# AILab-CVC/SEED-X

Hardware: AMD Instinct MI355X
Metric: end-to-end generations/sec (img-in -> txt + 1024px-img-out) (higher is better)
Workload: dtype fp16

## Files before the change

### seed-x_amd/csrc/gemm.hip

```cpp
#include "gemm_common.h"

namespace sxk_gemm {

template <typename TT, int BM, int BN, int WM, int WN, int NSTAGE, int AMODE>
__global__ __launch_bounds__(WM * WN * 64) void gemm_kernel(const GemmP p) {
#if defined(__HIP_DEVICE_COMPILE__)
  typedef typename TT::vec8 vec8;
  constexpr int NW = WM * WN;
  static_assert(NW == 4 || NW == 8, "4 or 8 waves per block");
  constexpr int TM = BM / WM, TN = BN / WN;
  constexpr int FM = TM / 16, FN = TN / 16;
  constexpr bool kGlu = (FN % 2 == 0);
  constexpr int BNP = (BN + 8 * NW - 1) / (8 * NW) * (8 * NW);
  constexpr int A_PER_WAVE = BM / (8 * NW);
  constexpr int B_PER_WAVE = BNP / (8 * NW);
  constexpr int LOADS = A_PER_WAVE + B_PER_WAVE;
  constexpr int A_BYTES = BM * 128, B_BYTES = BNP * 128, STAGE = A_BYTES + B_BYTES;
  static_assert(LOADS * (NSTAGE - 1) <= 63, "vmcnt range");
  extern __shared__ __attribute__((aligned(16))) unsigned char smem[];

  const int tid = threadIdx.x, lane = tid & 63;
  const int wave = __builtin_amdgcn_readfirstlane(tid >> 6);
  const int wm = wave / WN, wn = wave % WN;
  unsigned long long t_start = 0, t_first = 0, t_main = 0;
// ... 367 lines not shown
  SX_CHECK(a->M > 0 && a->N > 0 && a->K > 0, "sx_gemm: empty problem M=%d N=%d K=%d", a->M, a->N, a->K);
  SX_CHECK(a->K % 64 == 0, "sx_gemm: K=%d must be a multiple of 64 (pad the operand)", a->K);
  SX_CHECK(a->N % 16 == 0, "sx_gemm: N=%d must be a multiple of 16 (pad the weight)", a->N);
  SX_CHECK(!a->glu || a->N % 32 == 0, "sx_gemm: glu needs N %% 32 == 0");
  const int n_out = a->glu ? a->N / 2 : a->N;
  SX_CHECK(a->n_valid >= 0 && a->n_valid % 4 == 0 && a->n_valid <= n_out, "sx_gemm: n_valid=%d", a->n_valid);
  SX_CHECK(a->ldc >= (a->n_valid > 0 ? a->n_valid : n_out) && a->ldc % 4 == 0, "sx_gemm: ldc=%d invalid for n_out=%d",
           a->ldc, n_out);
  SX_CHECK(!a->residual || (a->ldr >= (a->n_valid > 0 ? a->n_valid : n_out) && a->ldr % 4 == 0), "sx_gemm: ldr=%d invalid", a->ldr);
  SX_CHECK(!a->bias2d || a->bias2d_rows > 0, "sx_gemm: bias2d_rows must be > 0");
  GemmP p;
  memset(&p, 0, sizeof(p));
  p.A = a->A; p.W = a->W; p.C = a->C; p.bias = a->bias; p.bias2d = a->bias2d; p.residual = a->residual;
  SX_CHECK(a->a_planes >= 0 && a->a_planes <= 2, "sx_gemm: a_planes=%d", a->a_planes);
  const int planes = a->a_planes == 2 ? 2 : 1;
  SX_CHECK(planes == 1 || (a->a_mode == SX_A_LINEAR && !ln), "sx_gemm: a_planes = 2 is for plain linear GEMMs");
  const int Kk = a->K * planes;
  p.M = a->M; p.N = a->N; p.K = Kk; p.Kw = a->K; p.ldc = a->ldc; p.ldr = a->ldr; p.res_mod = a->res_mod;
  p.n_valid = a->n_valid > 0 ? a->n_valid : n_out;
  p.bias2d_rows = a->bias2d_rows; p.out_dtype = a->out_dtype; p.act = a->act; p.glu = a->glu;
  p.ldb2 = a->ld_bias2d > 0 ? a->ld_bias2d : a->N;
  p.pad = 1;
  uint64_t a_bytes;
  if (a->a_mode == SX_A_CONV3X3) {
    SX_CHECK(a->Cin % 64 == 0 && a->K == 9 * a->Cin, "sx_gemm conv: Cin=%d K=%d", a->Cin, a->K);
    SX_CHECK(a->stride == 1 || a->stride == 2, "sx_gemm conv: stride");
    SX_CHECK(a->M == a->B * a->Hout * a->Wout, "sx_gemm conv: M != B*Hout*Wout");
    const int hv = a->upsample ? 2 * a->Hin : a->Hin, wv = a->upsample ? 2 * a->Win : a->Win;
    SX_CHECK(a->pad_mode == 0 || a->pad_mode == 1, "sx_gemm conv: pad_mode");
    const int padsum = a->pad_mode ? 1 : 2;
    SX_CHECK(a->Hout == (hv + padsum - 3) / a->stride + 1 && a->Wout == (wv + padsum - 3) / a->stride + 1,
             "sx_gemm conv: output geometry mismatch");
    p.pad = a->pad_mode ? 0 : 1;
    p.Hin = a->Hin; p.Win = a->Win; p.Cin = a->Cin; p.Hout = a->Hout; p.Wout = a->Wout;
    p.stride = a->stride; p.upsample = a->upsample;
    a_bytes = (uint64_t)a->B * a->Hin * a->Win * a->Cin * 2;
  } else {
    SX_CHECK(a->a_mode == SX_A_LINEAR, "sx_gemm: bad a_mode");
    a_bytes = (uint64_t)a->M * Kk * 2;
  }
  const uint64_t w_bytes = (uint64_t)a->N * a->K * 2;
  SX_CHECK(a_bytes < 0x7fffffffull && w_bytes < 0x7fffffffull, "sx_gemm: operand exceeds 2 GiB descriptor range");
  p.a_bytes = (unsigned)a_bytes;
  p.w_bytes = (unsigned)w_bytes;
  hipStream_t st = (hipStream_t)stream;
  p.res_init = (p.residual && p.act == SX_ACT_NONE && !p.glu) ? 1 : 0;
  if (ln) {
    SX_CHECK(a->a_mode == SX_A_LINEAR && !gn_stats, "sx_gemm_ln: linear GEMMs only");
    SX_CHECK(!(ln->row_stats_in && ln->row_stats_out), "sx_gemm_ln: a launch is a producer or a consumer, not both");
    if (ln->row_stats_out) {
      SX_CHECK(ln->x16_out && a->out_dtype == SX_F32 && !a->glu && a->act == SX_ACT_NONE && p.n_valid == a->N,
               "sx_gemm_ln producer: needs x16_out and a plain fp32 output of all N columns");
      SX_CHECK(ln->ld_x16 >= a->N && ln->ld_x16 % 4 == 0 && (((size_t)ln->x16_out) & 7) == 0, "sx_gemm_ln producer: ld_x16=%d", ln->ld_x16);
      p.ln_x16 = ln->x16_out; p.ln_ldx = ln->ld_x16; p.ln_out = ln->row_stats_out;
    } else {
      SX_CHECK(ln->colsum && ln->dim == a->K && ln->eps > 0.f, "sx_gemm_ln consumer: colsum / dim (= K) / eps");
      SX_CHECK(a->out_dtype == a->dtype && !a->residual && !a->bias2d, "sx_gemm_ln consumer: 16-bit output, no residual / bias2d");
      p.ln_in = ln->row_stats_in; p.ln_cs = ln->colsum; p.ln_eps = ln->eps; p.ln_inv_dim = 1.0f / (float)ln->dim;
    }
  }
  unsigned allow = 0x7f;
  if (ln) allow = 0;
  allow |= pp_supported(p, a->dtype, 256, a->a_mode) ? 0x80u : 0u;
  allow |= pp_supported(p, a->dtype, 320, a->a_mode) ? 0x100u : 0u;
  SX_CHECK(!(g_force_tile == 7 || g_force_tile == 8) || ((allow >> g_force_tile) & 1u),
           "sx_gemm: forced ping-pong tile has no kernel for this epilogue");
  if (ln) {
    const int plain = pick_tile(a->M, a->N, Kk, a->glu != 0, false, g_force_tile, 0x1ff);
    SX_CHECK((plain == 7 || plain == 8) && ((allow >> plain) & 1u),
             "sx_gemm_ln: M=%d N=%d K=%d does not run on a ping-pong tile with this epilogue (tile %d): keep sx_layernorm for it", a->M,
             a->N, a->K, plain);
    allow = 1u << plain;
  }
  const int cfg = pick_tile(a->M, a->N, Kk, a->glu != 0, a->a_mode == SX_A_CONV3X3, g_force_tile, allow);
  if (cfg == 7 || cfg == 8) {
    if (gn_stats && a->out_dtype == SX_F32 && !a->glu && a->act == SX_ACT_NONE && p.n_valid == a->N && a->N % gn_groups == 0 &&
        (a->N / gn_groups) % 2 == 0 && gn_rows % 256 == 0 && a->M % gn_rows == 0) {
      p.gn_stats = gn_stats; p.gn_groups = gn_groups; p.gn_cpg = a->N / gn_groups; p.gn_rows = gn_rows;
      *gn_fused = 1;
    }
    return launch_pp(p, a->dtype, cfg == 7 ? 256 : 320, a->a_mode, st);
  }
#define SX_GEMM_DISPATCH(TT)                                                  \
  switch (cfg) {                                                              \
    case 0: return launch_cfg<TT, 128, 128, 2, 2, 2>(p, a->a_mode, st);       \
    case 1: return launch_cfg<TT, 128, 80, 4, 1, 3>(p, a->a_mode, st);        \
    case 2: return launch_cfg<TT, 64, 128, 2, 2, 3>(p, a->a_mode, st);        \
    case 3: return launch_cfg<TT, 64, 64, 2, 2, 3>(p, a->a_mode, st);         \
    case 4: return launch_cfg<TT, 256, 256, 2, 4, 2>(p, a->a_mode, st);       \
    case 5: return launch_cfg<TT, 256, 320, 2, 4, 2>(p, a->a_mode, st);       \
    default: return launch_cfg<TT, 256, 160, 4, 2, 2>(p, a->a_mode, st);      \
  }
  if (a->dtype == SX_BF16) { SX_GEMM_DISPATCH(BF16) } else { SX_GEMM_DISPATCH(F16) }
#undef SX_GEMM_DISPATCH
}
```

### seed-x_amd/csrc/gemm_pp.hip

```cpp
#include "gemm_common.h"
#include <type_traits>

namespace sxk_gemm {

#define SX_A_CONV3X3_UP 2

#define PP_SYNC()                            \
  do {                                       \
    __builtin_amdgcn_sched_barrier(0);       \
    __builtin_amdgcn_s_barrier();            \
    __builtin_amdgcn_sched_barrier(0);       \
  } while (0)

template <typename TT, int BN, int AMODE, bool OUT32, int ACT, bool GLU, int LN = 0>
__global__ __launch_bounds__(512) void gemm_pp_kernel(const GemmP p) {
#if defined(__HIP_DEVICE_COMPILE__)
  typedef typename TT::vec8 vec8;
  static_assert(LN != 2 || (OUT32 && !GLU && ACT == SX_ACT_NONE), "the LayerNorm producer is the plain fp32-output epilogue");
  constexpr int BM = 256, TN = BN / 4, FN = TN / 16, FM = 8, FH = 4;
  constexpr int NB = BN / 64;
  constexpr int C1 = NB - 3, C2 = 3;
  constexpr int WAITN = 4 + NB;
  constexpr int A_BYTES = BM * 128, STAGE = A_BYTES + BN * 128;
  static_assert(!GLU || FN % 2 == 0, "GLU pairs n-fragments");
  static_assert(BN == 256 || BN == 320, "ping-pong tiles are 256x256 and 256x320");
  extern __shared__ __attribute__((aligned(16))) unsigned char smem[];

  const int tid = threadIdx.x, lane = tid & 63;
  const int wave = __builtin_amdgcn_readfirstlane(tid >> 6);
  const int g = wave >> 2, wc = wave & 3;
  unsigned long long t_start = 0, t_first = 0, t_main = 0;
  if (p.dbg) t_start = __builtin_amdgcn_s_memtime();

  int tile_m, tile_n;
  if (!tile_coords(p, blockIdx.x, gridDim.x, tile_m, tile_n)) return;
  const int m0 = tile_m * BM, n0 = tile_n * BN;

  double ln_s1 = 0.0, ln_s2 = 0.0;
  if constexpr (LN == 1) {
    if (tid < BM) {
      const int m = m0 + tid < p.M ? m0 + tid : p.M - 1;
      ln_s1 = p.ln_in[2 * (size_t)m];
      ln_s2 = p.ln_in[2 * (size_t)m + 1];
    }
  }
  __amdgpu_buffer_rsrc_t rA = __builtin_amdgcn_make_buffer_rsrc((void*)p.A, 0, (int)p.a_bytes, 0x00020000);
  __amdgpu_buffer_rsrc_t rW = __builtin_amdgcn_make_buffer_rsrc((void*)p.W, 0, (int)p.w_bytes, 0x00020000);

  const int rl = lane >> 3;
  const unsigned gchunk = ((lane & 7) ^ rl) << 4;
  unsigned a_off[4], a_msk[4];
  int a_lrow[4];
#pragma unroll
  for (int s = 0; s < 4; ++s) {
    a_lrow[s] = g * 128 + (s >> 1) * 64 + ((2 * wave + (s & 1)) & 7) * 8;
    const int row = m0 + a_lrow[s] + rl;
    if (AMODE == SX_A_LINEAR) {
      a_off[s] = (row < p.M) ? (unsigned)row * (unsigned)p.K * 2u + gchunk : 0xC0000000u;
      a_msk[s] = 0;
    } else {
      const int hw = p.Hout * p.Wout;
      const int b = row / hw, rem = row - b * hw;
      const int oy = rem / p.Wout, ox = rem - oy * p.Wout;
      const int Hv = p.upsample ? 2 * p.Hin : p.Hin, Wv = p.upsample ? 2 * p.Win : p.Win;
      const int vy = oy * p.stride - p.pad, vx = ox * p.stride - p.pad;
      unsigned msk = 0;
#pragma unroll
      for (int t = 0; t < 9; ++t) {
        const int iy = vy + t / 3, ix = vx + t % 3;
        if (row < p.M && iy >= 0 && iy < Hv && ix >= 0 && ix < Wv) msk |= 1u << t;
      }
      int sy = vy, sx = vx;
      if (AMODE == SX_A_CONV3X3_UP) {
        sy = oy >> 1; sx = ox >> 1;
        msk |= (unsigned)(oy & 1) << 9 | (unsigned)(ox & 1) << 10;
      }
      a_off[s] = (unsigned)(((b * p.Hin + sy) * p.Win + sx) * p.Cin) * 2u + gchunk;
      a_msk[s] = msk;
    }
  }
  unsigned w_off[NB];
#pragma unroll
  for (int i = 0; i < NB; ++i) {
    const int row = n0 + (wave * NB + i) * 8 + rl;
    w_off[i] = (row < p.N) ? (unsigned)row * (unsigned)p.Kw * 2u + gchunk : 0xC0000000u;
  }
  const int cpt = (AMODE != SX_A_LINEAR) ? p.Cin / 64 : 1;
  const int nkt = p.K / 64;
  const int nkw = p.Kw / 64;

  struct Tap { int cc, dy, dx; };
  auto tap_next = [&](Tap& t) {
    if (++t.cc == cpt) { t.cc = 0; if (++t.dx == 3) { t.dx = 0; ++t.dy; } }
  };

  auto koff_of = [&](int kt) -> unsigned { return (kt < nkt) ? (unsigned)kt * 128u : 0x80000000u; };
  auto koff_w = [&](int kt) -> unsigned { return (kt < nkt) ? (unsigned)(kt >= nkw ? kt - nkw : kt) * 128u : 0x80000000u; };
  auto dma_a = [&](int s, int buf, int kt, const Tap& t) {
    unsigned voff;
    if (AMODE == SX_A_LINEAR) {
      voff = a_off[s] + koff_of(kt);
    } else {
      const int tap = t.dy * 3 + t.dx;
      const bool ok = ((a_msk[s] >> tap) & 1u) != 0 && kt < nkt;
      unsigned o;
      if (AMODE == SX_A_CONV3X3_UP) {
        const int ry = ((int)((a_msk[s] >> 9) & 1u) + t.dy - 1) >> 1, rx = ((int)((a_msk[s] >> 10) & 1u) + t.dx - 1) >> 1;
        o = a_off[s] + (unsigned)((ry * p.Win + rx) * p.Cin) * 2u + (unsigned)t.cc * 128u;
      } else {
        o = a_off[s] + (unsigned)(((t.dy * p.Win + t.dx) * p.Cin + t.cc * 64) * 2);
      }
      voff = ok ? o : 0x80000000u;
    }
    __builtin_amdgcn_raw_ptr_buffer_load_lds(rA, SX_LDS_PTR(smem + buf * STAGE + a_lrow[s] * 128), 16, voff, 0, 0, 0);
  };
  auto dma_w = [&](int i, int buf, int kt) {
    __builtin_amdgcn_raw_ptr_buffer_load_lds(rW, SX_LDS_PTR(smem + buf * STAGE + A_BYTES + (wave * NB + i) * 1024), 16,
                                             w_off[i] + koff_w(kt), 0, 0, 0);
  };
  auto issue_x = [&](int buf, int kt, const Tap& t) {
    dma_a(0, buf, kt, t);
    dma_a(1, buf, kt, t);
#pragma unroll
    for (int i = 0; i < C1; ++i) dma_w(i, buf, kt);
  };
  auto issue_y = [&](int buf, int kt) {
// ... 112 lines not shown
    if (kt + 1 < nkt) ktile(std::integral_constant<int, 1>{}, kt + 1);
  }
  if (g == 0) PP_SYNC();
  wait_vmcnt<0>();

  if (p.dbg) t_main = __builtin_amdgcn_s_memtime();
  int ncol[FN], nout[FN];
  bool nok[FN];
  f32x4_t bv[FN];
#pragma unroll
  for (int i = 0; i < FN; ++i) {
    const int nb = n0 + wc * TN + i * 16;
    ncol[i] = nb + lq;
    nout[i] = GLU ? (nb >> 1) + lq : ncol[i];
    nok[i] = ncol[i] < p.N && nout[i] < p.n_valid && !(GLU && (i & 1));
    if (ncol[i] >= p.N) ncol[i] = p.N - 4;
    if (nout[i] + 4 > p.ldc) nout[i] = 0;
    bv[i] = (f32x4_t){0.f, 0.f, 0.f, 0.f};
  }
  if (p.bias) {
#pragma unroll
    for (int i = 0; i < FN; ++i) bv[i] = *(const f32x4_t*)(p.bias + ncol[i]);
  }
  const bool b2_uniform = p.bias2d && (m0 / p.bias2d_rows) == ((m0 + BM - 1 < p.M ? m0 + BM - 1 : p.M - 1) / p.bias2d_rows);
  if (b2_uniform) {
    const float* b2 = p.bias2d + (size_t)(m0 / p.bias2d_rows) * p.ldb2;
#pragma unroll
    for (int i = 0; i < FN; ++i) bv[i] += *(const f32x4_t*)(b2 + ncol[i]);
  }
  const bool b2_rows = p.bias2d && !b2_uniform;
  const bool res_late = p.residual && !p.res_init;
  const bool wide = !OUT32 && !GLU && (p.ldc & 7) == 0 && (((size_t)p.C) & 15) == 0;
  bool pair_ok[(FN + 1) / 2];
#pragma unroll
  for (int i = 0; i < (FN + 1) / 2; ++i) {
    const int lim = p.n_valid < p.N ? p.n_valid : p.N;
    pair_ok[i] = (2 * i + 1 < FN) && (n0 + wc * TN + i * 32 + 32 <= lim);
  }
  const bool glu_wide = GLU && !OUT32 && (p.ldc & 7) == 0 && (((size_t)p.C) & 15) == 0 &&
                        ((n0 + wc * TN) >> 1) + 32 <= (p.n_valid < (p.N >> 1) ? p.n_valid : (p.N >> 1));
  auto act1 = [&](f32x4_t x) -> f32x4_t {
    if (ACT == SX_ACT_GELU) {
      const f32x2_t g0 = gelu_erf2((f32x2_t){x[0], x[1]}), g1 = gelu_erf2((f32x2_t){x[2], x[3]});
      return (f32x4_t){g0[0], g0[1], g1[0], g1[1]};
    } else if (ACT == SX_ACT_SILU) {
      return (f32x4_t){silu_f(x[0]), silu_f(x[1]), silu_f(x[2]), silu_f(x[3])};
    }
    return x;
  };
  auto pack4 = [&](f32x4_t x) -> u32x2_t {
    u32x2_t o;
    o[0] = pack2<TT>(x[0], x[1]);
    o[1] = pack2<TT>(x[2], x[3]);
    return o;
  };
  f32x4_t lcs[LN == 1 ? FN : 1];
  if constexpr (LN == 1) {
#pragma unroll
    for (int i = 0; i < FN; ++i) lcs[i] = *(const f32x4_t*)(p.ln_cs + ncol[i]);
  }
  float lsum[LN == 2 ? FM : 1], lsq[LN == 2 ? FM : 1];
  const bool gn = OUT32 && p.gn_stats != nullptr;
  float gsl[FN], gql[FN], gsh[FN], gqh[FN];
#pragma unroll
  for (int i = 0; i < FN; ++i) gsl[i] = gql[i] = gsh[i] = gqh[i] = 0.f;
#pragma unroll
  for (int j = 0; j < FM; ++j) {
    const int m = m0 + g * 128 + j * 16 + (lane & 15);
    const bool mok = m < p.M;
    const int mc = mok ? m : p.M - 1;
    f32x4_t v[FN];
    if constexpr (LN == 1) {
      const f32x2_t ab = *(const f32x2_t*)(ln_lds + 2 * (g * 128 + j * 16 + (lane & 15)));
#pragma unroll
      for (int i = 0; i < FN; ++i) v[i] = acc[i][j] * ab[0] + (lcs[i] * ab[1] + bv[i]);
    } else {
#pragma unroll
      for (int i = 0; i < FN; ++i) v[i] = acc[i][j] + bv[i];
    }
    if (b2_rows) {
      const float* b2 = p.bias2d + (size_t)(mc / p.bias2d_rows) * p.ldb2;
#pragma unroll
      for (int i = 0; i < FN; ++i) v[i] += *(const f32x4_t*)(b2 + ncol[i]);
    }
    if (GLU) {
#pragma unroll
      for (int i = 0; i + 1 < FN; i += 2) {
        const f32x4_t gt = act1(v[i + 1]);
        v[i] = v[i] * gt;
      }
    } else if (ACT != SX_ACT_NONE) {
#pragma unroll
      for (int i = 0; i < FN; ++i) v[i] = act1(v[i]);
    }
    if (res_late) {
      const float* rr = p.residual + (size_t)(p.res_mod ? (mc % p.res_mod) : mc) * p.ldr;
#pragma unroll
      for (int i = 0; i < FN; ++i) {
        if (GLU && (i & 1)) continue;
        const int c = (nout[i] + 4 <= p.ldr) ? nout[i] : 0;
        v[i] += *(const f32x4_t*)(rr + c);
      }
    }
    if (OUT32) {
#pragma unroll
      for (int i = 0; i < FN; ++i)
        if (mok && nok[i]) *(f32x4_t*)((float*)p.C + (size_t)m * p.ldc + nout[i]) = v[i];
      if constexpr (LN == 2) {
        float s1 = 0.f, s2 = 0.f;
#pragma unroll
        for (int i = 0; i < FN; ++i) {
          if (mok && nok[i]) {
            s1 += (v[i][0] + v[i][1]) + (v[i][2] + v[i][3]);
            s2 += (v[i][0] * v[i][0] + v[i][1] * v[i][1]) + (v[i][2] * v[i][2] + v[i][3] * v[i][3]);
          }
        }
        lsum[j] = s1;
        lsq[j] = s2;
        const bool xwide = (p.ln_ldx & 7) == 0 && (((size_t)p.ln_x16) & 15) == 0;
#pragma unroll
        for (int i = 0; i < FN; ++i) {
          if ((i & 1) == 0 && i + 1 < FN && xwide && pair_ok[i >> 1]) {
            const u32x2_t o0 = pack4(v[i]), o1 = pack4(v[i + 1]);
            const auto w0 = __builtin_amdgcn_permlane16_swap(o0[0], o1[0], false, false);
            const auto w1 = __builtin_amdgcn_permlane16_swap(o0[1], o1[1], false, false);
            if (mok) {
              const u32x4_t w4 = {w0[0], w1[0], w0[1], w1[1]};
              const int q = lane >> 4;
              const int col = n0 + wc * TN + i * 16 + (q & 1) * 16 + (q >> 1) * 8;
              *(u32x4_t*)((unsigned short*)p.ln_x16 + (size_t)m * p.ln_ldx + col) = w4;
// ... 19 lines not shown
          const u32x2_t o0 = pack4(v[0]), o1 = pack4(v[2]);
          const auto s0 = __builtin_amdgcn_permlane16_swap(o0[0], o1[0], false, false);
          const auto s1 = __builtin_amdgcn_permlane16_swap(o0[1], o1[1], false, false);
          if (mok) {
            const u32x4_t w4 = {s0[0], s1[0], s0[1], s1[1]};
            const int q = lane >> 4;
            const int col = ((n0 + wc * TN) >> 1) + (q & 1) * 16 + (q >> 1) * 8;
            *(u32x4_t*)((unsigned short*)p.C + (size_t)m * p.ldc + col) = w4;
          }
          continue;
        }
      }
#pragma unroll
      for (int i = 0; i < FN; ++i) {
        if (GLU && (i & 1)) continue;
        if (!GLU && wide && (i & 1) == 0 && i + 1 < FN && pair_ok[i >> 1]) {
          const u32x2_t o0 = pack4(v[i]), o1 = pack4(v[i + 1]);
          const auto s0 = __builtin_amdgcn_permlane16_swap(o0[0], o1[0], false, false);
          const auto s1 = __builtin_amdgcn_permlane16_swap(o0[1], o1[1], false, false);
          if (mok) {
            const u32x4_t w4 = {s0[0], s1[0], s0[1], s1[1]};
            const int q = lane >> 4;
            const int col = n0 + wc * TN + i * 16 + (q & 1) * 16 + (q >> 1) * 8;
            *(u32x4_t*)((unsigned short*)p.C + (size_t)m * p.ldc + col) = w4;
          }
          continue;
        }
        if (!GLU && wide && (i & 1) && pair_ok[i >> 1]) continue;
        if (mok && nok[i]) *(u32x2_t*)((unsigned short*)p.C + (size_t)m * p.ldc + nout[i]) = pack4(v[i]);
      }
    }
  }
  if constexpr (LN == 2) {
    float* racc = (float*)smem;
    __syncthreads();
#pragma unroll
    for (int j = 0; j < FM; ++j) {
      float s1 = lsum[j], s2 = lsq[j];
      s1 += __shfl_xor(s1, 16, 64); s2 += __shfl_xor(s2, 16, 64);
      s1 += __shfl_xor(s1, 32, 64); s2 += __shfl_xor(s2, 32, 64);
      if (lane < 16) *(f32x2_t*)(racc + ((size_t)(wc * BM + g * 128 + j * 16 + lane)) * 2) = (f32x2_t){s1, s2};
    }
    __syncthreads();
    if (tid < BM && m0 + tid < p.M) {
      float s1 = 0.f, s2 = 0.f;
#pragma unroll
      for (int w = 0; w < 4; ++w) { s1 += racc[(w * BM + tid) * 2]; s2 += racc[(w * BM + tid) * 2 + 1]; }
      atomicAdd(&p.ln_out[2 * (size_t)(m0 + tid)], (double)s1);
      atomicAdd(&p.ln_out[2 * (size_t)(m0 + tid) + 1], (double)s2);
    }
  }
  if (OUT32 && gn) {
// ... 77 lines not shown
  if (p.glu) {
    if (out32) return -1;
    if (p.act == SX_ACT_GELU) return 2;
    if (p.act == SX_ACT_SILU) return 3;
    return -1;
  }
  if (p.act == SX_ACT_NONE) return out32 ? 4 : 0;
  if (p.act == SX_ACT_GELU && !out32) return 1;
  return -1;
}

bool pp_supported(const GemmP& p, int dtype, int bn, int a_mode) {
  const int e = epi_code(p, dtype);
  if (e < 0) return false;
  if (p.ln_in && !(a_mode == SX_A_LINEAR && (e == 0 || e == 2) && !p.ln_out)) return false;
  if (p.ln_out && !(a_mode == SX_A_LINEAR && e == 4 && !p.gn_stats)) return false;
  if (bn == 320 && (e == 2 || e == 3)) return false;
  if (a_mode == SX_A_CONV3X3 && !(e == 0 || e == 4)) return false;
  if (a_mode == SX_A_CONV3X3 && p.upsample && !(p.stride == 1 && p.pad == 1)) return false;
  return bn == 256 || bn == 320;
}

template <typename TT>
static int launch_t(const GemmP& p, int dtype, int bn, int a_mode, hipStream_t st) {
  const int e = epi_code(p, dtype);
#define PP_CASE(BNV, AM, O32, ACTV, GLUV) return launch_one<TT, BNV, AM, O32, ACTV, GLUV>(p, st)
  if (p.ln_in) {
    if (e == 2) return launch_one<TT, 256, SX_A_LINEAR, false, SX_ACT_GELU, true, 1>(p, st);
    if (bn == 256) return launch_one<TT, 256, SX_A_LINEAR, false, SX_ACT_NONE, false, 1>(p, st);
    return launch_one<TT, 320, SX_A_LINEAR, false, SX_ACT_NONE, false, 1>(p, st);
  }
  if (p.ln_out) {
    if (bn == 256) return launch_one<TT, 256, SX_A_LINEAR, true, SX_ACT_NONE, false, 2>(p, st);
    return launch_one<TT, 320, SX_A_LINEAR, true, SX_ACT_NONE, false, 2>(p, st);
  }
  if (a_mode == SX_A_LINEAR) {
    if (bn == 256) {
      switch (e) {
        case 0: PP_CASE(256, SX_A_LINEAR, false, SX_ACT_NONE, false);
        case 1: PP_CASE(256, SX_A_LINEAR, false, SX_ACT_GELU, false);
        case 2: PP_CASE(256, SX_A_LINEAR, false, SX_ACT_GELU, true);
        case 3: PP_CASE(256, SX_A_LINEAR, false, SX_ACT_SILU, true);
        case 4: PP_CASE(256, SX_A_LINEAR, true, SX_ACT_NONE, false);
      }
    } else {
      switch (e) {
        case 0: PP_CASE(320, SX_A_LINEAR, false, SX_ACT_NONE, false);
        case 1: PP_CASE(320, SX_A_LINEAR, false, SX_ACT_GELU, false);
// ... 39 lines not shown
```

### seed-x_amd/ops.py

```python
import contextlib
import ctypes as C
import gc
import math

import os

import torch

from . import _lib
from ._lib import (SX_A_CONV3X3, SX_A_LINEAR, SX_ACT_GELU, SX_ACT_NONE, SX_ACT_SILU, SX_BF16, SX_F16, SX_F32,
                   AttnArgs, AttnSmallArgs, GemmArgs, GemvArgs, check)

_DT = {torch.float16: SX_F16, torch.bfloat16: SX_BF16, torch.float32: SX_F32}
_TD = {v: k for k, v in _DT.items()}
ACT = {None: SX_ACT_NONE, "none": SX_ACT_NONE, "gelu": SX_ACT_GELU, "silu": SX_ACT_SILU}


def dt_code(dtype):
    return _DT[dtype]


def _stream():
    return C.c_void_p(torch.cuda.current_stream().cuda_stream)

# ... 111 lines not shown
    args.bias2d_rows = bias2d_rows
    args.dtype = _DT[a.dtype]
    args.out_dtype = _DT[out_dtype]
    args.act = ACT[act]
    args.glu = 1 if glu else 0
    args.a_mode = SX_A_LINEAR
    args.a_planes = a_planes
    if ln_emit is not None or ln_apply is not None:
        assert gn is None and not (ln_emit is not None and ln_apply is not None)
        la = _lib.GemmLnArgs()
        if ln_emit is not None:
            assert ln_emit.x16.shape == (M, N) and ln_emit.x16.dtype == a.dtype and ln_emit.stats.shape[0] == M
            la.x16_out, la.ld_x16, la.row_stats_out = ln_emit.x16.data_ptr(), ln_emit.x16.stride(0), ln_emit.stats.data_ptr()
        else:
            rows, colsum, eps = ln_apply
            assert rows.stats.shape[0] == M and colsum.dtype == torch.float32 and colsum.numel() == N and colsum.is_contiguous()
            la.row_stats_in, la.colsum, la.dim, la.eps = rows.stats.data_ptr(), colsum.data_ptr(), K, float(eps)
        check(lib.sx_gemm_ln(C.byref(args), C.byref(la), _stream()), "sx_gemm_ln")
        return out
    _launch_gemm(lib, args, gn, "sx_gemm")
    return out


def conv3x3(x, w, bias=None, bias2d=None, residual=None, stride=1, upsample=False, out_dtype=None, act=None,
            n_valid=0, pad_mode=0, gn=None):
    lib = _lib.load()
    assert x.dim() == 4 and x.is_contiguous() and w.is_contiguous()
    B, H, W, Cin = x.shape
    Cout, K = w.shape
    assert K == 9 * Cin
    hv, wv = (2 * H, 2 * W) if upsample else (H, W)
    padsum = 1 if pad_mode else 2
    Hout, Wout = (hv + padsum - 3) // stride + 1, (wv + padsum - 3) // stride + 1
    M = B * Hout * Wout
    out_dtype = out_dtype or x.dtype
    n_store = n_valid if n_valid else Cout
    out = torch.empty((M, n_store), dtype=out_dtype, device=x.device)
    args = GemmArgs()
    args.A, args.W, args.C = x.data_ptr(), w.data_ptr(), out.data_ptr()
    args.bias = _f32c(bias).data_ptr() if bias is not None else None
    args.n_valid = n_valid
    if bias2d is not None:
        assert bias2d.dtype == torch.float32 and bias2d.stride(-1) == 1 and bias2d.shape == (B, Cout)
        args.bias2d = bias2d.data_ptr()
        args.bias2d_rows = Hout * Wout
        args.ld_bias2d = bias2d.stride(0)
    if residual is not None:
        assert residual.dtype == torch.float32 and residual.stride(-1) == 1
        args.residual = residual.data_ptr()
        args.ldr = residual.stride(0)
    args.M, args.N, args.K = M, Cout, K
    args.ldc = n_store
    args.dtype = _DT[x.dtype]
    args.out_dtype = _DT[out_dtype]
    args.act = ACT[act]
    args.a_mode = SX_A_CONV3X3
    args.B, args.Hin, args.Win, args.Cin, args.Hout, args.Wout = B, H, W, Cin, Hout, Wout
    args.stride = stride
    args.upsample = 1 if upsample else 0
    args.pad_mode = pad_mode
    _launch_gemm(lib, args, gn, "sx_gemm(conv3x3)")
    return out.view(B, Hout * Wout, n_store)


def pack_decode_tiles(w):
    N, K = w.shape
    assert N % 16 == 0 and K % 32 == 0
    return w.view(N // 16, 16, K // 32, 32).permute(0, 2, 1, 3).contiguous().view(N, K)


def pack_decode_tiles20(w):
    N, K = w.shape
    assert N % 20 == 0 and K % 32 == 0
    return w.view(N // 20, 20, K // 32, 32).permute(0, 2, 1, 3).contiguous().view(N, K)


def _fp8_row_order(codes):
    K = codes.shape[-1]
    return codes.reshape(*codes.shape[:-1], K // 64, 2, 4, 8).transpose(-3, -2).reshape(*codes.shape[:-1], K // 64, 64)


def pack_decode_tiles_fp8(codes):
# ... 928 lines not shown
```

### seed-x_amd/unet.py

```python
import math
import os
import types

import torch

from . import ops
from .llama import glu_pack_rows

LN_FOLD = os.environ.get("SX_LN_FOLD", "1") != "0"

SDXL_BASE_CONFIG = dict(in_channels=4, out_channels=4, block_out_channels=(320, 640, 1280), layers_per_block=2,
                        down_attn=(False, True, True), up_attn=(True, True, False), transformer_layers=(1, 2, 10),
                        heads=(5, 10, 20), cross_attention_dim=2048, addition_time_embed_dim=256, pooled_dim=1280,
                        norm_groups=32, sample_size=128)


class UNetOutput:
    def __init__(self, sample):
        self.sample = sample


class UNet2DConditionModel:
    def __init__(self, comm=None, **cfg):
        from .parallel import Comm
# ... 165 lines not shown
        for i, co in enumerate(boc):
            blk = dict(res=[], attn=[], down=None)
            for j in range(c["layers_per_block"]):
                blk["res"].append(resnet(f"down_blocks.{i}.resnets.{j}"))
                if c["down_attn"][i]:
                    blk["attn"].append(transformer(f"down_blocks.{i}.attentions.{j}", c["transformer_layers"][i], c["heads"][i]))
            if i != len(boc) - 1:
                n = f"down_blocks.{i}.downsamplers.0.conv"
                blk["down"] = (conv16(n + ".weight"), f32(n + ".bias"))
            P["down"].append(blk)
        P["mid"] = dict(res=[resnet("mid_block.resnets.0")], attn=[transformer("mid_block.attentions.0", c["transformer_layers"][-1], c["heads"][-1])])
        P["mid"]["res"].append(resnet("mid_block.resnets.1"))
        P["up"] = []
        rh, rl = list(reversed(c["heads"])), list(reversed(c["transformer_layers"]))
        for i in range(len(boc)):
            blk = dict(res=[], attn=[], up=None)
            for j in range(c["layers_per_block"] + 1):
                blk["res"].append(resnet(f"up_blocks.{i}.resnets.{j}"))
                if c["up_attn"][i]:
                    blk["attn"].append(transformer(f"up_blocks.{i}.attentions.{j}", rl[i], rh[i]))
            if i != len(boc) - 1:
                n = f"up_blocks.{i}.upsamplers.0.conv"
                blk["up"] = (conv16(n + ".weight"), f32(n + ".bias"))
            P["up"].append(blk)
        P["norm_out"] = (f32("conv_norm_out.weight"), f32("conv_norm_out.bias"))
        wo = conv16("conv_out.weight")
        wop = torch.zeros(16, wo.shape[1], dtype=dt, device=dev)
        wop[:wo.shape[0]] = wo
        bo = torch.zeros(16, dtype=torch.float32, device=dev)
        bo[:wo.shape[0]] = f32("conv_out.bias")
        P["conv_out_w"], P["conv_out_b"] = wop, bo
        ws = [sd[n + ".time_emb_proj.weight"].detach().to(dev, dt) for n in self._temb_names]
        bs = [sd[n + ".time_emb_proj.bias"].detach().to(dev, torch.float32) for n in self._temb_names]
        P["temb_w"], P["temb_b"] = torch.cat(ws, 0).contiguous(), torch.cat(bs, 0).contiguous()
        off, P["temb_off"] = 0, {}
        for n, w_ in zip(self._temb_names, ws):
            P["temb_off"][n] = (off, w_.shape[0])
            off += w_.shape[0]
        self._P = P
        self._sd = None
        return P

    def _gn(self, x, gb, eps, silu, Hc, Wc, want_raw=False, x2=None, stats=None):
        G, dt = self.cfg["norm_groups"], self.dtype
        return ops.groupnorm(x, gb[0], gb[1], G, eps, silu, dt, want_raw=want_raw, x2=x2, comm=self.comm, hw_total=Hc * Wc,
                             stats=stats)

    def _gn_slot(self, B, HW):
        if self._gn_arena is None:
            return None
        i = self._gn_next
        self._gn_next += 1
        if i >= self._gn_arena.shape[0]:
            return None
        return ops.GnStats(self._gn_arena[i], self.cfg["norm_groups"], HW)

    def _conv(self, h16, B, Hc, Wc, w, bias=None, bias2d=None, residual=None, stride=1, upsample=False, n_valid=0, gn=None):
        tp = self.comm.world
        Cin = h16.shape[-1]
        if tp == 1:
            return ops.conv3x3(h16.view(B, Hc, Wc, Cin), w, bias=bias, bias2d=bias2d, residual=residual, stride=stride,
                               upsample=upsample, out_dtype=torch.float32, n_valid=n_valid, gn=gn)
        from . import seqpar
        Hl = Hc // tp
        Co = n_valid or w.shape[0]
        if stride == 2:
            xin = seqpar.with_halo(h16, self.comm, Hl, Wc, left_col=True, bottom=False)
            out = ops.conv3x3(xin, w, bias=bias, bias2d=bias2d, stride=2, pad_mode=1, out_dtype=torch.float32)
            assert residual is None
            return out.view(B, (Hl // 2) * (Wc // 2), Co)
        xin = seqpar.with_halo(h16, self.comm, Hl, Wc)
        out = ops.conv3x3(xin, w, bias=bias, bias2d=bias2d, upsample=upsample, out_dtype=torch.float32, n_valid=n_valid)
        f = 2 if upsample else 1
        out = out.view(B, f * (Hl + 2), f * Wc, Co)[:, f:f * (Hl + 1)].reshape(B, f * Hl * f * Wc, Co).contiguous()
        if residual is not None:
            out = ops.add(out, residual.reshape(out.shape).contiguous())
        return out

    def _resnet(self, r, x, B, Hc, Wc, temb_all, skip=None, st_in=None):
        Ci = x.shape[-1] + (skip.shape[-1] if skip is not None else 0)
        if "ws" in r:
            h, raw = self._gn(x, r["n1"], 1e-5, True, Hc, Wc, want_raw=True, x2=skip)
        else:
            assert skip is None
            h = self._gn(x, r["n1"], 1e-5, True, Hc, Wc, stats=st_in)
# ... 150 lines not shown
            for j, r in enumerate(blk["res"]):
                x, st = self._resnet(r, x, B, Hc, Wc, temb_all, st_in=st)
                if blk["attn"]:
                    x, st = self._transformer(blk["attn"][j], x, B, ctx[ti], Hc, Wc, st_in=st)
                    ti += 1
                skips.append((x, Hc, Wc))
            if blk["down"] is not None:
                st = self._gn_slot(B, (Hc // 2) * (Wc // 2))
                x = self._conv(ops.cast(x, dt), B, Hc, Wc, blk["down"][0], bias=blk["down"][1], stride=2, gn=st)
                Hc, Wc = Hc // 2, Wc // 2
                skips.append((x, Hc, Wc))
        x, st = self._resnet(P["mid"]["res"][0], x, B, Hc, Wc, temb_all, st_in=st)
        x, st = self._transformer(P["mid"]["attn"][0], x, B, ctx[ti], Hc, Wc, st_in=st)
        ti += 1
        x, st = self._resnet(P["mid"]["res"][1], x, B, Hc, Wc, temb_all, st_in=st)
        for blk in P["up"]:
            for j, r in enumerate(blk["res"]):
                s, _, _ = skips.pop()
                x, st = self._resnet(r, x.contiguous(), B, Hc, Wc, temb_all, skip=s)
                if blk["attn"]:
                    x, st = self._transformer(blk["attn"][j], x, B, ctx[ti], Hc, Wc, st_in=st)
                    ti += 1
            if blk["up"] is not None:
                x = self._conv(ops.cast(x, dt), B, Hc, Wc, blk["up"][0], bias=blk["up"][1], upsample=True)
                Hc, Wc = Hc * 2, Wc * 2
                st = None
        h = self._gn(x, P["norm_out"], 1e-5, True, Hc, Wc, stats=st)
        self._gn_arena = None
        self._on_mark = None
        nv = 4 if c["out_channels"] == 4 else 0
        out = self._conv(h, B, Hc, Wc, P["conv_out_w"], bias=P["conv_out_b"], n_valid=nv)
        out = out.view(B, -1, out.shape[-1])
        if tp > 1:
            out = seqpar.gather_rows(out, self.comm)
            if not torch.cuda.is_current_stream_capturing():
                self.comm.check()
        return out

    def forward(self, sample, timestep, encoder_hidden_states, added_cond_kwargs=None, cross_attention_kwargs=None,
                return_dict=True, **_):
        self._pack()
        assert added_cond_kwargs is not None and "text_embeds" in added_cond_kwargs and "time_ids" in added_cond_kwargs
        B, Cin, H, W = sample.shape
        assert Cin == self.cfg["in_channels"]
        dev = self.device
        t = torch.as_tensor(timestep, dtype=torch.float32, device=dev).reshape(-1)
        t = t.expand(B).contiguous() if t.numel() == 1 else t
# ... 11 lines not shown
```

### seed-x_amd/vae.py

```python
import json
import math
import os
from types import SimpleNamespace

import torch

from . import ops

EPS = 1e-6


def pack_planes(w32, taps=1, role="w"):
    w3 = w32.reshape(w32.shape[0], taps, -1)
    hi = w3.to(torch.bfloat16)
    lo = (w3 - hi.float()).to(torch.bfloat16)
    planes = [hi, lo, hi] if role == "w" else [hi, hi, lo]
    return torch.cat(planes, dim=2).reshape(w32.shape[0], -1).contiguous()


class DecoderOutput:
    def __init__(self, sample):
        self.sample = sample


# ... 208 lines not shown

        lc, boc = c.latent_channels, c.block_out_channels
        assert lc == 4, "post_quant_conv / conv_in packing assumes 4 latent channels"
        top = boc[-1]
        P = {}
        bpq = torch.zeros(16, dtype=torch.float32, device=dev)
        bpq[:lc] = f32("post_quant_conv.bias")
        P["pq"] = (padded(f32("post_quant_conv.weight").reshape(lc, lc), 16, 64), bpq)
        self.cin_kpad = (9 * lc + 63) // 64 * 64
        P["conv_in"] = (padded(conv32("decoder.conv_in.weight"), top, self.cin_kpad), f32("decoder.conv_in.bias"))
        a = "decoder.mid_block.attentions.0."
        P["mid"] = dict(r0=resnet("decoder.mid_block.resnets.0"), r1=resnet("decoder.mid_block.resnets.1"),
                        gn=(f32(a + "group_norm.weight"), f32(a + "group_norm.bias")),
                        wq=lin16(a + "to_q.weight"), bq=f32(a + "to_q.bias"),
                        wk=lin16(a + "to_k.weight"), bk=f32(a + "to_k.bias"),
                        wv=lin16(a + "to_v.weight", role="a"), bv=f32(a + "to_v.bias"),
                        wo=lin16(a + "to_out.0.weight"), bo=f32(a + "to_out.0.bias"))
        P["up"] = []
        for i in range(len(boc)):
            blk = dict(res=[resnet(f"decoder.up_blocks.{i}.resnets.{j}") for j in range(c.layers_per_block + 1)], up=None)
            if i != len(boc) - 1:
                n = f"decoder.up_blocks.{i}.upsamplers.0.conv"
                blk["up"] = (conv16(n + ".weight"), f32(n + ".bias"))
            P["up"].append(blk)
        P["norm_out"] = (f32("decoder.conv_norm_out.weight"), f32("decoder.conv_norm_out.bias"))
        wo = conv32("decoder.conv_out.weight")
        bo = torch.zeros(16, dtype=torch.float32, device=dev)
        bo[:wo.shape[0]] = f32("decoder.conv_out.bias")
        if two:
            w16 = torch.zeros(16, 9, wo.shape[1] // 9, dtype=torch.float16, device=dev)
            w16[:wo.shape[0]] = wo.reshape(wo.shape[0], 9, -1).to(torch.float16)
            P["conv_out"] = (torch.cat([w16, w16], dim=2).reshape(16, -1).contiguous(), bo)
        else:
            P["conv_out"] = (padded(wo, 16, wo.shape[1], taps=9), bo)
        P["p_out"] = (2 if two else 3) if split else 1
        P["two"] = two
        if self.has_encoder:
            E = {}
            ci = c.in_channels
            self.enc_kpad = (9 * ci + 63) // 64 * 64
            E["conv_in"] = (padded(conv32("encoder.conv_in.weight"), boc[0], self.enc_kpad), f32("encoder.conv_in.bias"))
            E["down"] = []
            for i in range(len(boc)):
                blk = dict(res=[resnet(f"encoder.down_blocks.{i}.resnets.{j}") for j in range(c.layers_per_block)], down=None)
                if i != len(boc) - 1:
                    n = f"encoder.down_blocks.{i}.downsamplers.0.conv"
# ... 80 lines not shown
    def _im2col(self, x, kpad):
        if not self.split:
            return ops.im2col3x3_small(x, kpad, self.operand_dtype)
        pl = ops.split_bf16(x.view(-1, 4))
        hi, lo = (ops.im2col3x3_small(ops.cast(pl[:, a:a + 4].contiguous(), torch.float32).view(x.shape), kpad,
                                      torch.bfloat16) for a in (0, 8))
        return torch.cat([hi, hi, lo], dim=1)

    def _decode_one(self, z_nchw):
        P, c, f32 = self._P, self.config, torch.float32
        _, lc, h, w = z_nchw.shape
        zp = ops.nchw_to_nhwc(z_nchw, ld=64)
        x = ops.gemm(self._A(zp.view(-1, 64)), P["pq"][0], bias=P["pq"][1], out_dtype=f32, n_valid=4)
        col = self._im2col(x.view(1, h, w, lc), self.cin_kpad)
        x = ops.gemm(col, P["conv_in"][0], bias=P["conv_in"][1], out_dtype=f32).view(1, h * w, -1)
        x = self._resnet(P["mid"]["r0"], x, h, w)
        x = self._mid_attention(P["mid"], x)
        x = self._resnet(P["mid"]["r1"], x, h, w)
        H, W = h, w
        for blk in P["up"]:
            for r in blk["res"]:
                x = self._resnet(r, x, H, W)
            if blk["up"] is not None:
                x = ops.conv3x3(self._A(x).view(1, H, W, -1), blk["up"][0], bias=blk["up"][1], upsample=True, out_dtype=f32)
                H, W = 2 * H, 2 * W
        hN = self._gn(x, P["norm_out"], True, planes=P["p_out"])
        y = self._conv(P["p_out"], hN.view(1, H, W, -1), P["conv_out"][0], bias=P["conv_out"][1], out_dtype=f32,
                       n_valid=4)
        return ops.nhwc_to_nchw(y, c.out_channels, H, W)

    @torch.no_grad()
    def decode(self, z, return_dict=True, generator=None):
        self._pack()
        z = z.to(device=self.device, dtype=torch.float32)
        ops.OPERAND_PLANES = 3 if self.split else 1
        try:
            out = torch.cat([self._decode_one(z[b:b + 1].contiguous()) for b in range(z.shape[0])], dim=0)
        finally:
            ops.OPERAND_PLANES = 1
        return DecoderOutput(out) if return_dict else (out,)

    def _encode_one(self, img_nchw):
        P, c, f32 = self._P, self.config, torch.float32
        E = P["enc"]
        _, ci, H, W = img_nchw.shape
        nb = len(c.block_out_channels)
        assert H % (1 << (nb - 1)) == 0 and W % (1 << (nb - 1)) == 0
# ... 37 lines not shown
```

Baseline: 1.330.

## Decompose upsample+3x3 conv into four 2x2 sub-pixel phase convolutions

Nearest-neighbour 2x upsample followed by a 3x3 conv is rewritten as four phase-specific 2x2 convolutions over the low-resolution input. The kernel gains a new A-mode that gathers 4 taps instead of 9 and selects a per-phase weight slice. Output rows are scattered to their interleaved positions. This cuts the reduction length and the A-gather work for the upsampler convs in the UNet and VAE decoder. In exchange it adds pre-summed weights, which change rounding, plus extra weight memory and a constraint that the tile not straddle phases.

After: 1.352 (median of 6 runs). 1.7% higher.

```diff
diff --git a/seed-x_amd/csrc/gemm.hip b/seed-x_amd/csrc/gemm.hip
--- a/seed-x_amd/csrc/gemm.hip
+++ b/seed-x_amd/csrc/gemm.hip
@@ -413,9 +413,18 @@
   p.ldb2 = a->ld_bias2d > 0 ? a->ld_bias2d : a->N;
   p.pad = 1;
   uint64_t a_bytes;
+  const bool phases = a->a_mode == SX_A_CONV3X3 && a->upsample == 2;
   if (a->a_mode == SX_A_CONV3X3) {
-    SX_CHECK(a->Cin % 64 == 0 && a->K == 9 * a->Cin, "sx_gemm conv: Cin=%d K=%d", a->Cin, a->K);
+    SX_CHECK(a->upsample >= 0 && a->upsample <= 2, "sx_gemm conv: upsample=%d", a->upsample);
+    SX_CHECK(a->Cin % 64 == 0 && a->K == (phases ? 4 : 9) * a->Cin, "sx_gemm conv: Cin=%d K=%d", a->Cin, a->K);
     SX_CHECK(a->stride == 1 || a->stride == 2, "sx_gemm conv: stride");
+    if (phases) {
+      SX_CHECK(a->stride == 1 && a->pad_mode == 0, "sx_gemm conv: upsample = 2 is stride 1, pad 1");
+      SX_CHECK((int64_t)a->B * a->Hin * a->Win % 256 == 0,
+               "sx_gemm conv: upsample = 2 needs B*Hin*Win %% 256 == 0 (B=%d Hin=%d Win=%d): a 256-row tile must not straddle a phase",
+               a->B, a->Hin, a->Win);
+      SX_CHECK(!a->residual && !gn_stats, "sx_gemm conv: upsample = 2 takes no residual and no GroupNorm statistics");
+    }
     SX_CHECK(a->M == a->B * a->Hout * a->Wout, "sx_gemm conv: M != B*Hout*Wout");
     const int hv = a->upsample ? 2 * a->Hin : a->Hin, wv = a->upsample ? 2 * a->Win : a->Win;
     SX_CHECK(a->pad_mode == 0 || a->pad_mode == 1, "sx_gemm conv: pad_mode");
@@ -430,7 +439,7 @@
     SX_CHECK(a->a_mode == SX_A_LINEAR, "sx_gemm: bad a_mode");
     a_bytes = (uint64_t)a->M * Kk * 2;
   }
-  const uint64_t w_bytes = (uint64_t)a->N * a->K * 2;
+  const uint64_t w_bytes = (uint64_t)a->N * a->K * 2 * (phases ? 4 : 1);
   SX_CHECK(a_bytes < 0x7fffffffull && w_bytes < 0x7fffffffull, "sx_gemm: operand exceeds 2 GiB descriptor range");
   p.a_bytes = (unsigned)a_bytes;
   p.w_bytes = (unsigned)w_bytes;
@@ -451,7 +460,7 @@
     }
   }
   unsigned allow = 0x7f;
-  if (ln) allow = 0;
+  if (ln || phases) allow = 0;
   allow |= pp_supported(p, a->dtype, 256, a->a_mode) ? 0x80u : 0u;
   allow |= pp_supported(p, a->dtype, 320, a->a_mode) ? 0x100u : 0u;
   SX_CHECK(!(g_force_tile == 7 || g_force_tile == 8) || ((allow >> g_force_tile) & 1u),
@@ -463,7 +472,9 @@
              a->N, a->K, plain);
     allow = 1u << plain;
   }
-  const int cfg = pick_tile(a->M, a->N, Kk, a->glu != 0, a->a_mode == SX_A_CONV3X3, g_force_tile, allow);
+  SX_CHECK(!phases || allow, "sx_gemm conv: upsample = 2 has no ping-pong kernel for this epilogue");
+  const int force = (phases && g_force_tile != 7 && g_force_tile != 8) ? -1 : g_force_tile;
+  const int cfg = pick_tile(a->M, a->N, Kk, a->glu != 0, a->a_mode == SX_A_CONV3X3, force, allow);
   if (cfg == 7 || cfg == 8) {
     if (gn_stats && a->out_dtype == SX_F32 && !a->glu && a->act == SX_ACT_NONE && p.n_valid == a->N && a->N % gn_groups == 0 &&
         (a->N / gn_groups) % 2 == 0 && gn_rows % 256 == 0 && a->M % gn_rows == 0) {
diff --git a/seed-x_amd/csrc/gemm_pp.hip b/seed-x_amd/csrc/gemm_pp.hip
--- a/seed-x_amd/csrc/gemm_pp.hip
+++ b/seed-x_amd/csrc/gemm_pp.hip
@@ -4,6 +4,7 @@
 namespace sxk_gemm {
 
 #define SX_A_CONV3X3_UP 2
+#define SX_A_CONV3X3_PH 3
 
 #define PP_SYNC()                            \
   do {                                       \
@@ -35,6 +36,7 @@
   int tile_m, tile_n;
   if (!tile_coords(p, blockIdx.x, gridDim.x, tile_m, tile_n)) return;
   const int m0 = tile_m * BM, n0 = tile_n * BN;
+  const int ph = (AMODE == SX_A_CONV3X3_PH) ? m0 / (p.M >> 2) : 0;
 
   double ln_s1 = 0.0, ln_s2 = 0.0;
   if constexpr (LN == 1) {
@@ -58,6 +60,18 @@
     if (AMODE == SX_A_LINEAR) {
       a_off[s] = (row < p.M) ? (unsigned)row * (unsigned)p.K * 2u + gchunk : 0xC0000000u;
       a_msk[s] = 0;
+    } else if (AMODE == SX_A_CONV3X3_PH) {
+      const int r = row - ph * (p.M >> 2);
+      const int q = r / p.Win, j = r - q * p.Win, i = q % p.Hin;
+      const int sy = i + (ph >> 1) - 1, sx = j + (ph & 1) - 1;
+      unsigned msk = 0;
+#pragma unroll
+      for (int t = 0; t < 4; ++t) {
+        const int iy = sy + (t >> 1), ix = sx + (t & 1);
+        if (row < p.M && iy >= 0 && iy < p.Hin && ix >= 0 && ix < p.Win) msk |= 1u << t;
+      }
+      a_off[s] = (unsigned)((r + ((ph >> 1) - 1) * p.Win + (ph & 1) - 1) * p.Cin) * 2u + gchunk;
+      a_msk[s] = msk;
     } else {
       const int hw = p.Hout * p.Wout;
       const int b = row / hw, rem = row - b * hw;
@@ -80,18 +94,20 @@
     }
   }
   unsigned w_off[NB];
+  const unsigned w_ph = (unsigned)ph * (unsigned)p.N * (unsigned)p.Kw * 2u;
 #pragma unroll
   for (int i = 0; i < NB; ++i) {
     const int row = n0 + (wave * NB + i) * 8 + rl;
-    w_off[i] = (row < p.N) ? (unsigned)row * (unsigned)p.Kw * 2u + gchunk : 0xC0000000u;
+    w_off[i] = (row < p.N) ? w_ph + (unsigned)row * (unsigned)p.Kw * 2u + gchunk : 0xC0000000u;
   }
   const int cpt = (AMODE != SX_A_LINEAR) ? p.Cin / 64 : 1;
   const int nkt = p.K / 64;
   const int nkw = p.Kw / 64;
 
   struct Tap { int cc, dy, dx; };
+  constexpr int TW = (AMODE == SX_A_CONV3X3_PH) ? 2 : 3;
   auto tap_next = [&](Tap& t) {
-    if (++t.cc == cpt) { t.cc = 0; if (++t.dx == 3) { t.dx = 0; ++t.dy; } }
+    if (++t.cc == cpt) { t.cc = 0; if (++t.dx == TW) { t.dx = 0; ++t.dy; } }
   };
 
   auto koff_of = [&](int kt) -> unsigned { return (kt < nkt) ? (unsigned)kt * 128u : 0x80000000u; };
@@ -101,7 +117,7 @@
     if (AMODE == SX_A_LINEAR) {
       voff = a_off[s] + koff_of(kt);
     } else {
-      const int tap = t.dy * 3 + t.dx;
+      const int tap = t.dy * TW + t.dx;
       const bool ok = ((a_msk[s] >> tap) & 1u) != 0 && kt < nkt;
       unsigned o;
       if (AMODE == SX_A_CONV3X3_UP) {
@@ -260,9 +276,15 @@
 #pragma unroll
     for (int i = 0; i < FN; ++i) bv[i] = *(const f32x4_t*)(p.bias + ncol[i]);
   }
-  const bool b2_uniform = p.bias2d && (m0 / p.bias2d_rows) == ((m0 + BM - 1 < p.M ? m0 + BM - 1 : p.M - 1) / p.bias2d_rows);
+  auto out_row = [&](int m) -> int {
+    if (AMODE != SX_A_CONV3X3_PH) return m;
+    const int r = m - ph * (p.M >> 2);
+    const int q = r / p.Win, j = r - q * p.Win;
+    return (2 * q + (ph >> 1)) * p.Wout + 2 * j + (ph & 1);
+  };
+  const bool b2_uniform = p.bias2d && (out_row(m0) / p.bias2d_rows) == (out_row(m0 + BM - 1 < p.M ? m0 + BM - 1 : p.M - 1) / p.bias2d_rows);
   if (b2_uniform) {
-    const float* b2 = p.bias2d + (size_t)(m0 / p.bias2d_rows) * p.ldb2;
+    const float* b2 = p.bias2d + (size_t)(out_row(m0) / p.bias2d_rows) * p.ldb2;
 #pragma unroll
     for (int i = 0; i < FN; ++i) bv[i] += *(const f32x4_t*)(b2 + ncol[i]);
   }
@@ -307,6 +329,7 @@
     const int m = m0 + g * 128 + j * 16 + (lane & 15);
     const bool mok = m < p.M;
     const int mc = mok ? m : p.M - 1;
+    const int mo = out_row(m);
     f32x4_t v[FN];
     if constexpr (LN == 1) {
       const f32x2_t ab = *(const f32x2_t*)(ln_lds + 2 * (g * 128 + j * 16 + (lane & 15)));
@@ -317,7 +340,7 @@
       for (int i = 0; i < FN; ++i) v[i] = acc[i][j] + bv[i];
     }
     if (b2_rows) {
-      const float* b2 = p.bias2d + (size_t)(mc / p.bias2d_rows) * p.ldb2;
+      const float* b2 = p.bias2d + (size_t)(out_row(mc) / p.bias2d_rows) * p.ldb2;
 #pragma unroll
       for (int i = 0; i < FN; ++i) v[i] += *(const f32x4_t*)(b2 + ncol[i]);
     }
@@ -343,7 +366,7 @@
     if (OUT32) {
 #pragma unroll
       for (int i = 0; i < FN; ++i)
-        if (mok && nok[i]) *(f32x4_t*)((float*)p.C + (size_t)m * p.ldc + nout[i]) = v[i];
+        if (mok && nok[i]) *(f32x4_t*)((float*)p.C + (size_t)mo * p.ldc + nout[i]) = v[i];
       if constexpr (LN == 2) {
         float s1 = 0.f, s2 = 0.f;
 #pragma unroll
@@ -409,12 +432,12 @@
             const u32x4_t w4 = {s0[0], s1[0], s0[1], s1[1]};
             const int q = lane >> 4;
             const int col = n0 + wc * TN + i * 16 + (q & 1) * 16 + (q >> 1) * 8;
-            *(u32x4_t*)((unsigned short*)p.C + (size_t)m * p.ldc + col) = w4;
+            *(u32x4_t*)((unsigned short*)p.C + (size_t)mo * p.ldc + col) = w4;
           }
           continue;
         }
         if (!GLU && wide && (i & 1) && pair_ok[i >> 1]) continue;
-        if (mok && nok[i]) *(u32x2_t*)((unsigned short*)p.C + (size_t)m * p.ldc + nout[i]) = pack4(v[i]);
+        if (mok && nok[i]) *(u32x2_t*)((unsigned short*)p.C + (size_t)mo * p.ldc + nout[i]) = pack4(v[i]);
       }
     }
   }
@@ -538,8 +561,23 @@
 }
 
 template <typename TT>
+static int launch_phases(const GemmP& p, int e, int bn, hipStream_t st) {
+#define PH_CASE(BNV, O32) return launch_one<TT, BNV, SX_A_CONV3X3_PH, O32, SX_ACT_NONE, false>(p, st)
+  if (bn == 256) {
+    if (e == 0) PH_CASE(256, false);
+    if (e == 4) PH_CASE(256, true);
+  } else {
+    if (e == 0) PH_CASE(320, false);
+    if (e == 4) PH_CASE(320, true);
+  }
+#undef PH_CASE
+  return -1;
+}
+
+template <typename TT>
 static int launch_t(const GemmP& p, int dtype, int bn, int a_mode, hipStream_t st) {
   const int e = epi_code(p, dtype);
+  if (a_mode == SX_A_CONV3X3 && p.upsample == 2) return launch_phases<TT>(p, e, bn, st);
 #define PP_CASE(BNV, AM, O32, ACTV, GLUV) return launch_one<TT, BNV, AM, O32, ACTV, GLUV>(p, st)
   if (p.ln_in) {
     if (e == 2) return launch_one<TT, 256, SX_A_LINEAR, false, SX_ACT_GELU, true, 1>(p, st);
diff --git a/seed-x_amd/ops.py b/seed-x_amd/ops.py
--- a/seed-x_amd/ops.py
+++ b/seed-x_amd/ops.py
@@ -157,20 +157,59 @@
     return out
 
 
+_PHASE_TAPS = {(0, 0): (0,), (0, 1): (1, 2), (1, 0): (0, 1), (1, 1): (2,)}
+
+
+def pack_upsample_phases(w, planes=1, dtype=None, rounded=True):
+    assert w.dim() == 2 and w.shape[1] % 9 == 0 and planes in (1, 3)
+    Cout, C = w.shape[0], w.shape[1] // 9
+    w9 = w.detach().double().reshape(Cout, 3, 3, C)
+    wp = torch.zeros((4, Cout, 2, 2, C), dtype=torch.float64, device=w.device)
+    for (a, u), kys in _PHASE_TAPS.items():
+        for (c, v), kxs in _PHASE_TAPS.items():
+            for ky in kys:
+                for kx in kxs:
+                    wp[2 * a + c, :, u, v] += w9[:, ky, kx]
+    if not rounded:
+        assert planes == 1
+        return wp.view(4, Cout, 4 * C)
+    if planes == 1:
+        return wp.to(dtype or w.dtype).view(4, Cout, 4 * C).contiguous()
+    s32 = wp.float()
+    hi = s32.to(torch.bfloat16)
+    lo = (s32 - hi.float()).to(torch.bfloat16)
+    return torch.cat([hi, lo, hi], dim=4).view(4, Cout, 12 * C).contiguous()
+
+
+def upsample_phases_ok(B, H, W):
+    return (B * H * W) % 256 == 0
+
+
 def conv3x3(x, w, bias=None, bias2d=None, residual=None, stride=1, upsample=False, out_dtype=None, act=None,
-            n_valid=0, pad_mode=0, gn=None):
-    lib = _lib.load()
-    assert x.dim() == 4 and x.is_contiguous() and w.is_contiguous()
+            n_valid=0, pad_mode=0, gn=None, w_phases=None, out=None):
+    lib = _lib.load()
+    assert x.dim() == 4 and x.is_contiguous()
     B, H, W, Cin = x.shape
-    Cout, K = w.shape
-    assert K == 9 * Cin
+    phases = (w_phases is not None and upsample and stride == 1 and pad_mode == 0 and residual is None and gn is None
+              and act is None and upsample_phases_ok(B, H, W))
+    if phases:
+        assert w_phases.dim() == 3 and w_phases.shape[0] == 4 and w_phases.shape[2] == 4 * Cin and w_phases.dtype == x.dtype
+        w = w_phases
+        Cout, K = w.shape[1], 4 * Cin
+    else:
+        assert w is not None, "conv3x3: this call needs the 36-tap weight (the phase gate does not hold)"
+        Cout, K = w.shape
+        assert K == 9 * Cin
+    assert w.is_contiguous()
     hv, wv = (2 * H, 2 * W) if upsample else (H, W)
     padsum = 1 if pad_mode else 2
     Hout, Wout = (hv + padsum - 3) // stride + 1, (wv + padsum - 3) // stride + 1
     M = B * Hout * Wout
     out_dtype = out_dtype or x.dtype
     n_store = n_valid if n_valid else Cout
-    out = torch.empty((M, n_store), dtype=out_dtype, device=x.device)
+    if out is None:
+        out = torch.empty((M, n_store), dtype=out_dtype, device=x.device)
+    assert out.shape == (M, n_store) and out.dtype == out_dtype and out.is_contiguous()
     args = GemmArgs()
     args.A, args.W, args.C = x.data_ptr(), w.data_ptr(), out.data_ptr()
     args.bias = _f32c(bias).data_ptr() if bias is not None else None
@@ -192,7 +231,7 @@
     args.a_mode = SX_A_CONV3X3
     args.B, args.Hin, args.Win, args.Cin, args.Hout, args.Wout = B, H, W, Cin, Hout, Wout
     args.stride = stride
-    args.upsample = 1 if upsample else 0
+    args.upsample = (2 if phases else 1) if upsample else 0
     args.pad_mode = pad_mode
     _launch_gemm(lib, args, gn, "sx_gemm(conv3x3)")
     return out.view(B, Hout * Wout, n_store)
diff --git a/seed-x_amd/unet.py b/seed-x_amd/unet.py
--- a/seed-x_amd/unet.py
+++ b/seed-x_amd/unet.py
@@ -211,6 +211,8 @@
             if i != len(boc) - 1:
                 n = f"up_blocks.{i}.upsamplers.0.conv"
                 blk["up"] = (conv16(n + ".weight"), f32(n + ".bias"))
+                w = sd[n + ".weight"].detach().to(dev)
+                blk["up_ph"] = ops.pack_upsample_phases(w.permute(0, 2, 3, 1).reshape(w.shape[0], -1), dtype=dt)
             P["up"].append(blk)
         P["norm_out"] = (f32("conv_norm_out.weight"), f32("conv_norm_out.bias"))
         wo = conv16("conv_out.weight")
@@ -244,12 +246,13 @@
             return None
         return ops.GnStats(self._gn_arena[i], self.cfg["norm_groups"], HW)
 
-    def _conv(self, h16, B, Hc, Wc, w, bias=None, bias2d=None, residual=None, stride=1, upsample=False, n_valid=0, gn=None):
+    def _conv(self, h16, B, Hc, Wc, w, bias=None, bias2d=None, residual=None, stride=1, upsample=False, n_valid=0, gn=None,
+              w_phases=None):
         tp = self.comm.world
         Cin = h16.shape[-1]
         if tp == 1:
             return ops.conv3x3(h16.view(B, Hc, Wc, Cin), w, bias=bias, bias2d=bias2d, residual=residual, stride=stride,
-                               upsample=upsample, out_dtype=torch.float32, n_valid=n_valid, gn=gn)
+                               upsample=upsample, out_dtype=torch.float32, n_valid=n_valid, gn=gn, w_phases=w_phases)
         from . import seqpar
         Hl = Hc // tp
         Co = n_valid or w.shape[0]
@@ -446,7 +449,7 @@
                     x, st = self._transformer(blk["attn"][j], x, B, ctx[ti], Hc, Wc, st_in=st)
                     ti += 1
             if blk["up"] is not None:
-                x = self._conv(ops.cast(x, dt), B, Hc, Wc, blk["up"][0], bias=blk["up"][1], upsample=True)
+                x = self._conv(ops.cast(x, dt), B, Hc, Wc, blk["up"][0], bias=blk["up"][1], upsample=True, w_phases=blk["up_ph"])
                 Hc, Wc = Hc * 2, Wc * 2
                 st = None
         h = self._gn(x, P["norm_out"], 1e-5, True, Hc, Wc, stats=st)
diff --git a/seed-x_amd/vae.py b/seed-x_amd/vae.py
--- a/seed-x_amd/vae.py
+++ b/seed-x_amd/vae.py
@@ -254,6 +254,7 @@
             if i != len(boc) - 1:
                 n = f"decoder.up_blocks.{i}.upsamplers.0.conv"
                 blk["up"] = (conv16(n + ".weight"), f32(n + ".bias"))
+                blk["up_ph"] = ops.pack_upsample_phases(conv32(n + ".weight"), planes=3 if split else 1, dtype=dt)
             P["up"].append(blk)
         P["norm_out"] = (f32("decoder.conv_norm_out.weight"), f32("decoder.conv_norm_out.bias"))
         wo = conv32("decoder.conv_out.weight")
@@ -380,7 +381,8 @@
             for r in blk["res"]:
                 x = self._resnet(r, x, H, W)
             if blk["up"] is not None:
-                x = ops.conv3x3(self._A(x).view(1, H, W, -1), blk["up"][0], bias=blk["up"][1], upsample=True, out_dtype=f32)
+                x = ops.conv3x3(self._A(x).view(1, H, W, -1), blk["up"][0], bias=blk["up"][1], upsample=True, out_dtype=f32,
+                                w_phases=blk["up_ph"])
                 H, W = 2 * H, 2 * W
         hN = self._gn(x, P["norm_out"], True, planes=P["p_out"])
         y = self._conv(P["p_out"], hN.view(1, H, W, -1), P["conv_out"][0], bias=P["conv_out"][1], out_dtype=f32,
```
